# chriskery/slurm-bridge-operator

Hardware: AMD Instinct MI355X
Metric: placements/sec + job×node fit evals/sec, 100k nodes×1M jobs, 1–8 MI355X (higher is better)
Workload: dtype int32

## Files before the change

slurm-bridge-operator_amd/csrc/dev_decider_bench.hip:

```cpp
#define MW_DECIDER_BENCH 1
#include "fit_commit_mw.h"

namespace fitgpu {
__global__ __launch_bounds__(64) void k_dec_bench(int w, int32_t* out, unsigned long long* cyc) {
    extern __shared__ __attribute__((aligned(16))) unsigned char smem[];
    MwShared* S = reinterpret_cast<MwShared*>(smem);
    const int lane = threadIdx.x;
    mw_reset_items(S, threadIdx.x);
    __syncthreads();
    for (int r = 0; r < MW_R; ++r) {
        if (lane == 0) {
            S->rec[r].h = MwHdr{0u, 1, MW_M, r, 1, 1, 0, 0, 1u, 0u, KEY_INF};
        }
        if (lane < MW_M) {
            const int s = r * MW_M + lane;
            S->rec[r].it[lane] = MwItem{(uint32_t)s, (uint32_t)(lane + 1), s, s, 1000000, 1000000, 0, 0, 1u,
                                        mw_lds_addr(&S->rows[s].ver), 0xffffffffu, 1u};
            S->rows[s] = MwRow{1000000, 1000000, 0, 0, 1u, (uint32_t)s, s, 0};
        }
    }
    for (int i = lane; i < 64; i += 64) S->bitmap[i] = 0u;
    if (lane == 0) S->dn = 0ull;
    __syncthreads();
    CompPlan P{};
    P.nb = 0;
    P.ne = 2048;
    P.w = w;
    const unsigned long long t0 = __builtin_amdgcn_s_memtime();
    const CommitResult r = mw_decider(P, S, out, 1);
    const unsigned long long t1 = __builtin_amdgcn_s_memtime();
    if (lane == 0) {
        cyc[0] = t1 - t0;
        cyc[1] = r.done;
        cyc[2] = r.placed;
        cyc[3] = r.dirty;
    }
}
}

extern "C" int dec_bench(int w, unsigned long long* host_out) {
    int32_t* out;
    unsigned long long* cyc;
    if (hipMalloc(&out, sizeof(int32_t) * (w + 64)) != hipSuccess) return -1;
    if (hipMalloc(&cyc, 64) != hipSuccess) return -1;
// ... 12 lines not shown
```

slurm-bridge-operator_amd/csrc/engine.cpp:

```cpp
#include <errno.h>
#include <fcntl.h>
#include <hip/hip_runtime_api.h>
#include <hip/hip_vector_types.h>
#include <rccl/rccl.h>
#include <sys/file.h>
#include <sys/stat.h>
#include <unistd.h>

#include <algorithm>
#include <chrono>
#include <cstdarg>
#include <cstdio>
#include <cstdlib>
#include <cstring>
#include <initializer_list>
#include <map>
#include <mutex>
#include <new>
#include <string>
#include <vector>

#include "../../include/fitgpu.h"
#include "fit_device.h"

// ... 278 lines not shown
    DBuf<NodeRec> rec;
    DBuf<int32_t> col_cpu, col_mem, col_gpu, col_av, perm;
    DBuf<uint32_t> col_mask;
    DBuf<int32_t> rb_cpu, rb_mem, rb_gpu;
    std::vector<uint32_t> h_mask;
    bool have_nodes = false;
    int64_t loads = 0;

    int32_t np = 0;
    int32_t ptab[128];
    DBuf<int32_t> d_ptab;

    DBuf<int32_t> jcpu, jmem, jgpu, jwall, out, jl, jpk;
    DBuf<uint16_t> jpart, jk;
    DBuf<int8_t> jcomp;
    DBuf<uint64_t> cand, bnd;
    DBuf<JobRec> wjob;
    DBuf<CompPlan> plan;
    DBuf<CommitResult> res;
    HBuf<CompPlan> h_plan;
    HBuf<CommitResult> h_res;
    DBuf<int32_t> jls;
    HBuf<int32_t> h_jls;

    int32_t tl_slots = 0, tl_slot_min = 0;
    bool have_tl = false;
    DBuf<Seg> slab;
    DBuf<TlHdr> tlhdr;
    DBuf<int32_t> outs, rel_off, rel_slot, rel_cpu, rel_mem, rel_gpu;
    DBuf<uint32_t> tl_err;
// ... 272 lines not shown
    int rc = engine_plan(c, jb, E, (int64_t)MAX_SLICES * KS, [&](int32_t len, CompState& s) {
        for (s.ks = KS;; s.ks /= 2) {
            const int slices = MAX_SLICES * KS / s.ks;
            s.sub = std::max(MIN_SUB, (len + SCAN_WAVES * slices - 1) / (SCAN_WAVES * slices));
            s.nslice = std::max(1, (len + SCAN_WAVES * s.sub - 1) / (SCAN_WAVES * s.sub));
            if (s.sub <= sub_target || s.ks / 2 < ks_min) break;
        }
    });
    if (rc) return rc;
    size_t lds = engine_lds_bytes(E.maxnodes);
    if (const char* e = getenv("FIT_ENGINE_LDS_MIN")) lds = std::max(lds, (size_t)atol(e));
    int per_cu = engine_blocks_per_cu(lds);
    if (per_cu <= 0) return fail(FIT_E_HIP, "k_engine does not fit on a CU (lds %zu)", lds);
    int workers = std::max(8, std::max(1, per_cu - 1) * c->cus - nc);
    if (const char* e = getenv("FIT_WORKERS")) workers = std::max(1, atoi(e));
    static const bool no_backup = getenv("FIT_REC_BACKUP") && atoi(getenv("FIT_REC_BACKUP")) == 0;
    if (c->rec_bak.ensure(std::max(c->nn, 1))) return FIT_E_OOM;
    if (!no_backup)
        HIP_TRY(hipMemcpyAsync(c->rec_bak.p, c->rec.p, sizeof(NodeRec) * c->nn, hipMemcpyDeviceToDevice, st));
    return engine_launch(
        c, jb, E, workers, "placement engine",
        [&]() -> int {
            HIP_TRY(launch_engine(nc + workers, lds, st, c->ectl.p, c->ering.p, c->ecs.p, c->eco.p,
                                  c->plan.p, nc, c->rec.p, c->jl.p, cpu, mem, gpu, wall, part, nk,
                                  c->cand.p, c->bnd.p, c->wjob.p, out, kmax, c->ebusy.p, c->jpk.p,
                                  c->wd_ticks));
            return 0;
        },
        [&](int trip) -> int {
            if (!trip) return 0;
            if (no_backup) {
                c->have_nodes = c->have_tl = false;
                return trip;
            }
            HIP_TRY(hipMemcpyAsync(c->rec.p, c->rec_bak.p, sizeof(NodeRec) * c->nn, hipMemcpyDeviceToDevice, st));
            HIP_TRY(hipStreamSynchronize(st));
            return trip;
        },
        S);
}

// ... 248 lines not shown
               const SmallBatch* hb = nullptr) {
    const double t0 = now_ms();
    fit_stats S;
    memset(&S, 0, sizeof S);
    S.jobs = J;
    hipStream_t st = c->st;
    if (J <= c->small_direct && !c->collective()) {
        const int rc = place_direct(c, J, cpu, mem, gpu, wall, part, nk, kmax, out, h_out, S, hb);
        if (rc) return rc;
        if (h_out_done) *h_out_done = h_out != nullptr;
        S.unplaced = J - S.placed - S.rejected;
        S.ms_total = now_ms() - t0;
        if (stats) *stats = S;
        return 0;
    }
    if (c->jcomp.ensure(std::max(J, 1))) return FIT_E_OOM;
    HIP_TRY(launch_prefilter(st, cpu, mem, gpu, wall, part, nk, J, kmax, c->d_ptab.p, c->np, out,
                             c->jcomp.p));
    const int C = c->ncomp;
    std::vector<int32_t> jb;
    const int pre_mode = !c->collective() ? 0
                         : (c->shard_mode == FIT_SHARD_AUTO ? (C >= c->world ? FIT_SHARD_COMPONENTS : FIT_SHARD_NODES)
                                                            : c->shard_mode);
    const bool cls_able = c->cls_nodes_ok && pre_mode != FIT_SHARD_NODES;
    const bool try_cls = (c->cls_mode == 1 || c->cls_mode == 2) && cls_able && (c->cls_mode == 2 || J > c->small_batch);
    bool cls_ok = false;
    int rc0 = build_job_lists(c, J, S, jb, cpu, mem, gpu, part, try_cls, &cls_ok);
    if (rc0) return rc0;
    const int32_t live = J - S.rejected;
    if (c->cls_mode == 3 && cls_able && live > c->small_batch && 2 * (int64_t)c->last_multi >= live) {
        rc0 = classify_jobs(c, J, cpu, mem, gpu, part, &cls_ok);
        if (rc0) return rc0;
    }
// ... 1389 lines not shown
```

slurm-bridge-operator_amd/csrc/fit_commit_mw.h:

```cpp
#pragma once
#include "fit_common.h"
#include "fit_engine_ctl.h"

namespace fitgpu {

#ifndef MW_ITEMS
#define MW_ITEMS 8
#endif
constexpr int MW_M = MW_ITEMS;
constexpr int MW_R = 8;
#ifndef MW_SNAP
#define MW_SNAP MW_ITEMS
#endif
static_assert(MW_SNAP >= 1 && MW_SNAP <= MW_ITEMS, "a later snapshot only shortens the ring span");
constexpr int MW_WAVES = SCAN_WAVES;
constexpr int MW_H = MW_WAVES - 1;
static_assert(MW_M == 8, "the decider holds one item per lane of its 8-lane ring group");
static_assert(MW_R >= MW_M, "record slot reuse relies on the lag bound");

#ifndef MW_HSLEEP
#define MW_HSLEEP 1
#endif
constexpr int MW_EPL = (MAX_SLICES * KS + 63) / 64;
static_assert(MW_EPL <= 2, "at most two candidate entries per lane");

struct alignas(16) MwRow {
    int32_t cpu, mem, gpu, avail;
    uint32_t mask, pos;
    int32_t orig, ver;
};

struct alignas(16) MwItem {
    uint32_t pos, score;
    int32_t tag, orig;
    int32_t cpu, mem, gpu, avail;
    uint32_t mask;
    uint32_t chk_addr, chk_mask, chk_thr;
};

struct alignas(16) MwHdr {
    uint32_t ready;
    int32_t v, n, q;
    int32_t cpu, mem, gpu, wall;
    uint32_t pbit;
// ... 2 lines not shown
};

struct alignas(16) MwRec {
    MwHdr h;
    MwItem it[MW_M];
};

struct alignas(16) MwShared {
    uint64_t dn;
    uint32_t halt;
    uint32_t fail;
    int32_t res[4];
    uint32_t pubt;
    uint32_t wd;
    uint32_t trip_arg;
    uint32_t pad[5];
    MwRec rec[MW_R];
    MwRow rows[UCAP];
    uint32_t bitmap[1];
};

__host__ __device__ constexpr size_t mw_lds_bytes(int32_t max_component_nodes) {
    return sizeof(MwShared) + (size_t)((max_component_nodes + 31) / 32) * 4;
}

#ifdef FIT_STAMPS
constexpr int MW_NSTAMP = 24;
__device__ unsigned long long g_mw[64][MW_NSTAMP];
#define MW_CLK(v) unsigned long long v = __builtin_amdgcn_s_memtime()
#define MW_DECL(v) unsigned long long v = 0
#define MW_ACC(v, x) v += (x)
#define MW_ADD(I_, V_) do { if ((threadIdx.x & 63) == 0) atomicAdd(&g_mw[blockIdx.x & 63][I_], (unsigned long long)(V_)); } while (0)
#else
#define MW_CLK(v)
#define MW_DECL(v)
// ... 308 lines not shown
    return true;
}

template <class Q>
__device__ __forceinline__ Q* rfl_ptr(Q* p) {
    const uint64_t v = (uint64_t)(uintptr_t)p;
    return (Q*)(uintptr_t)(((uint64_t)(uint32_t)rfl((int32_t)(v >> 32)) << 32) |
                           (uint32_t)rfl((int32_t)(uint32_t)v));
}
__device__ __forceinline__ MwTiles tiles_sgpr(const MwTiles& T) {
    return MwTiles{rfl_ptr(T.tdone), (unsigned)rfl((int32_t)T.need), rfl_ptr(T.ring),
                   rfl_ptr(T.ctl), (unsigned)rfl((int32_t)T.round), (unsigned)rfl((int32_t)T.comp),
                   (unsigned)rfl((int32_t)T.ntj), rfl_ptr(T.feas)};
}

constexpr int UPL_MW = UCAP / 64;
constexpr int MW_NE = MW_EPL + UPL_MW;
static_assert(MW_NE <= 8, "entry index takes 3 bits (and 4 bits of item index each in 32)");
static_assert(MW_M <= 15, "item index + 1 fits 4 bits");
__device__ __forceinline__ uint64_t mw_tag(uint64_t k, int e) {
    return k == KEY_INF ? KEY_INF
                        : (k & 0xffffffff00000000ull) | (uint32_t)(((uint32_t)k << 3) | (uint32_t)e);
}
__device__ __forceinline__ void mw_cas(uint64_t& a, uint64_t& b) {
    const uint64_t lo = umin64(a, b), hi = umax64(a, b);
    a = lo;
    b = hi;
}
template <int N>
__device__ __forceinline__ void mw_sort(uint64_t (&q)[N]) {
    if constexpr (N == 4) {
        mw_cas(q[0], q[1]); mw_cas(q[2], q[3]);
        mw_cas(q[0], q[2]); mw_cas(q[1], q[3]);
// ... 173 lines not shown
            R_->h.v = (int32_t)v_;                                                             \
            R_->h.n = n_;                                                                      \
            R_->h.q = J_.q;                                                                    \
            lds_release();                         \
            lds_st(&R_->h.ready, (uint32_t)i + 1u);                                            \
        }                                                                                      \
        {                                                                                      \
            MW_CLK(hp1_);                                                                      \
            MW_ACC(a_hp, hp1_);                                                                \
        }                                                                                      \
        MW_ACC(a_hn, 1);                                                                       \
        MW_ACC(a_hi, n_);                                                                      \
        i += MW_H;                                                                             \
    }

__device__ __noinline__ void mw_helper(const CompPlan& Pref, MwShared* Sin,
                                       const NodeRec* __restrict__ rec_,
                                       const uint64_t* __restrict__ cand_,
                                       const uint64_t* __restrict__ bnd_,
                                       const JobRec* __restrict__ wjob_, int h, MwTiles Tin) {
    const MwTiles T = tiles_sgpr(Tin);
    const GAS NodeRec* const rec = gview(rec_);
    const GAS uint64_t* const cand = gview(cand_);
    const GAS uint64_t* const bnd = gview(bnd_);
    const GAS JobRec* const wjob = gview(wjob_);
    const CompPlan P = plan_sgpr(Pref);
    MwShared* const S = lds_opaque(Sin);
    const int lane = threadIdx.x & 63;
    const int E = P.nslice * P.ks;
    bool has[MW_EPL];
    int64_t eoff[MW_EPL];
#pragma unroll
    for (int e = 0; e < MW_EPL; ++e) {
        has[e] = lane + 64 * e < E;
        eoff[e] = P.cand_off + (has[e] ? lane + 64 * e : 0);
// ... 60 lines not shown
    v4i32 a;
    v4i32 b;
    int32_t slot;
};

typedef uint32_t v4u32 __attribute__((ext_vector_type(4)));
struct MwRecRegs {
    v4u32 h0, h1, h2;
    v4u32 i0, i1, i2;
};

struct MwDec {
    int t, nu, placed, stop;
    int done;
    bool exit;
#ifdef MW_SEGSTAMP
    unsigned long long seg[8], prev;
#endif
};
#ifdef MW_SEGSTAMP
__device__ unsigned long long g_seg[8];
#define MW_SEG(D_, i)                                                                           \
    do {                                                                                        \
        __builtin_amdgcn_sched_barrier(0);                                                      \
        unsigned long long now_;                                                                \
        asm volatile("s_memtime %0\n\ts_waitcnt lgkmcnt(0)" : "=s"(now_)::"memory");            \
        __builtin_amdgcn_sched_barrier(0);                                                      \
        if (i > 0) D_.seg[i] += now_ - D_.prev;                                                 \
        D_.prev = now_;                                                                         \
    } while (0)
// ... 11 lines not shown
    x.h1 = hp[1];
    x.h2 = hp[2];
    x.i0 = ip[0];
    x.i1 = ip[1];
    x.i2 = ip[2];
}

__device__ __forceinline__ void mw_reset_items(MwShared* S, unsigned tid) {
    static_assert(sizeof(MwItem) == 48 && offsetof(MwItem, mask) == 32, "the probe is the last 16 B");
    static_assert((MW_M & (MW_M - 1)) == 0, "item index by shift and mask");
    const uint32_t sink = mw_lds_addr(&S->pad[0]);
    for (unsigned i = tid; i < MW_R * MW_M; i += blockDim.x)
        *reinterpret_cast<v4u32*>(&S->rec[i / MW_M].it[i % MW_M].mask) = v4u32{0u, sink, 0u, 0u};
}

template <int E>
__device__ __forceinline__ void mw_decide(MwShared* S, const CompPlan& P, MwDec& D, MwRing& R,
                                          MwRecRegs& cur, MwRecRegs& nxt, uint32_t& flag,
                                          int32_t& oq, int32_t& ov, int32_t* out, int kmax,
                                          uint64_t& waitcyc) {
    const int lane = threadIdx.x & 63;
    const int t = D.t;
#ifdef MW_DECIDER_BENCH
    if (t >= P.w) D.exit = true;
#endif
    MW_SEG(D, 0);
    lds_release();
    __hip_atomic_store(&S->dn, ((uint64_t)(uint32_t)D.nu << 32) | (uint32_t)t, __ATOMIC_RELAXED,
                       __HIP_MEMORY_SCOPE_WORKGROUP);
    const MwRec* Rn = &S->rec[(E + 1) & (MW_R - 1)];
    const uint32_t flag_n = lds_ld(&Rn->h.ready);
// ... 27 lines not shown
        d.sm = (tr ? R.a.y : (int32_t)x.i1.y) - jm;
        d.sg = (tr ? R.a.z : (int32_t)x.i1.z) - jg;
        d.sa = tr ? R.a.w : (int32_t)x.i1.w;
        d.sk = tr ? R.b.x : (int32_t)x.i2.x;
        d.so = tr ? R.b.z : (int32_t)x.i0.w;
        d.ss = tr ? R.slot : (int32_t)x.i0.z;
        const uint64_t best = min8_2pass(cand);
        const uint64_t mine = __ballot(cand == best) & 0xffull;
        d.w = __builtin_ctzll(mine | 0x100ull) & 7;
        const uint32_t bhi = (uint32_t)readlane((int32_t)(best >> 32), 0);
        const uint32_t blo = (uint32_t)readlane((int32_t)(uint32_t)best, 0);
        d.bs = ((uint64_t)bhi << 32) | blo;
        d.placed = d.bs != KEY_INF;
        d.wslot = readlane(d.ss, d.w);
        d.fresh = d.placed && d.wslot < 0;
        d.full = d.fresh && D.nu >= UCAP;
        d.stopB = B != KEY_INF && d.bs > B;
        return d;
    };
    Dec d = decide(cur);
    MW_SEG(D, 2);
#ifdef MW_DECIDER_BENCH
    const bool rec_missing = false;
#else
    const bool rec_missing = flag != (uint32_t)t + 1u;
#endif
    if (__builtin_expect(!D.exit && (rec_missing || d.stopB || d.full), 0)) {
        if (rec_missing) {
            MW_CLK(c0);
            for (unsigned sp = 0;; ++sp) {
                flag = lds_ld(&S->rec[t & (MW_R - 1)].h.ready);
// ... 1 lines not shown
                if (sp > MW_SPIN_LIMIT || lds_ld(&S->fail)) {
                    lds_st(&S->fail, TRIP_DECIDER_REC);
                    D.stop = 3;
                    D.exit = true;
                    break;
                }
                __builtin_amdgcn_s_sleep(0);
            }
            lds_acquire();
            mw_read_rec(&S->rec[t & (MW_R - 1)], lane & 7, cur);
            {
                MW_CLK(c1);
                MW_ACC(waitcyc, c1 - c0);
            }
            d = decide(cur);
        }
        if (!D.exit && (d.stopB || d.full)) {
            D.done = (int32_t)cur.h2.y;
            if (D.done < P.w) D.stop = d.stopB ? 1 : 2;
            D.exit = true;
        }
    }
    MW_SEG(D, 3);
    const bool go = !D.exit;
    const bool placed = d.placed && go, fresh = d.fresh && go;
    const int w = d.w;
    const int32_t pos = (int32_t)(uint32_t)d.bs;
    const int32_t nc = readlane(d.sc, w), nm = readlane(d.sm, w), ng = readlane(d.sg, w);
    const int32_t na = readlane(d.sa, w), nk = readlane(d.sk, w), no = readlane(d.so, w);
    const int32_t slot = fresh ? D.nu : d.wslot;
// ... 34 lines not shown
            : "memory");
    }
    D.nu += fresh;
    D.placed += placed;
    MW_SEG(D, 6);
    oq = writelane(rfl((int32_t)cur.h0.w), t & 63, oq);
    ov = writelane(placed ? no : -1, t & 63, ov);
    if (E == 7 && go && (t & 63) == 63) {
        if (oq >= 0) ((GAS int32_t*)out)[(int64_t)oq * kmax] = ov;
        oq = -1;
    }
    D.t = t + (go ? 1 : 0);
    MW_SEG(D, 7);
}

__device__ __noinline__ CommitResult mw_decider(const CompPlan& Pref, MwShared* Sin,
                                                int32_t* __restrict__ out, int kmax) {
    const CompPlan P = plan_sgpr(Pref);
    MwShared* const S = lds_opaque(Sin);
    const int lane = threadIdx.x & 63;
    __builtin_amdgcn_s_setprio(3);
    MwDec D{0, 0, 0, 0, 0, false};
#ifdef MW_SEGSTAMP
    for (int i = 0; i < 8; ++i) D.seg[i] = 0;
    D.prev = 0;
#endif
    MwRing R;
    R.a = v4i32{0, 0, 0, 0};
    R.b = v4i32{0, -1, -1, -1};
    R.slot = -1;
    int32_t oq = -1, ov = -1;
    uint64_t waitcyc = 0;
    MW_CLK(d0);
    MwRecRegs ra, rb;
    uint32_t flag = 0;
    if (P.w > 0) {
        for (unsigned sp = 0;; ++sp) {
// ... 9 lines not shown
                break;
            }
            __builtin_amdgcn_s_sleep(0);
        }
        lds_acquire();
        mw_read_rec(&S->rec[0], lane & 7, ra);
    } else {
        D.exit = true;
    }
    {
        MW_CLK(r0c);
        MW_ADD(17, r0c - d0);
        MW_ADD(18, 1);
    }
    while (!D.exit) {
        mw_decide<0>(S, P, D, R, ra, rb, flag, oq, ov, out, kmax, waitcyc);
        mw_decide<1>(S, P, D, R, rb, ra, flag, oq, ov, out, kmax, waitcyc);
        mw_decide<2>(S, P, D, R, ra, rb, flag, oq, ov, out, kmax, waitcyc);
        mw_decide<3>(S, P, D, R, rb, ra, flag, oq, ov, out, kmax, waitcyc);
        mw_decide<4>(S, P, D, R, ra, rb, flag, oq, ov, out, kmax, waitcyc);
        mw_decide<5>(S, P, D, R, rb, ra, flag, oq, ov, out, kmax, waitcyc);
        mw_decide<6>(S, P, D, R, ra, rb, flag, oq, ov, out, kmax, waitcyc);
        mw_decide<7>(S, P, D, R, rb, ra, flag, oq, ov, out, kmax, waitcyc);
    }
    const int t = D.t;
    if (oq >= 0 && lane < (t & 63)) ((GAS int32_t*)out)[(int64_t)oq * kmax] = ov;
    lds_release();
    __hip_atomic_store(&S->dn, ((uint64_t)(uint32_t)D.nu << 32) | (uint32_t)t, __ATOMIC_RELAXED,
                       __HIP_MEMORY_SCOPE_WORKGROUP);
    lds_st(&S->halt, 1u);
    MW_CLK(d1);
    MW_ADD(0, d1 - d0);
#ifdef MW_SEGSTAMP
    if (lane == 0)
        for (int i = 0; i < 8; ++i) g_seg[i] = D.seg[i];
#endif
    MW_ADD(1, waitcyc);
    MW_ADD(2, t);
#ifdef MW_DECIDER_BENCH
    D.done = t;
#endif
    return CommitResult{D.done, D.stop, D.nu, D.placed};
}

// ... 1 lines not shown
                                                         NodeRec* __restrict__ rec,
                                                         const uint64_t* __restrict__ cand,
                                                         const uint64_t* __restrict__ bnd,
                                                         const JobRec* __restrict__ wjob,
                                                         int32_t* __restrict__ out, int kmax,
                                                         MwTiles T = MwTiles{nullptr, 0u, nullptr, nullptr, 0u, 0u, 0u, nullptr}) {
    const int wave = __builtin_amdgcn_readfirstlane((int)(threadIdx.x >> 6));
    const int nwords = (P.ne - P.nb + 31) >> 5;
    for (int i = threadIdx.x; i < nwords; i += MW_WAVES * 64) S->bitmap[i] = 0u;
    if (threadIdx.x < MW_R) S->rec[threadIdx.x].h.ready = 0u;
    mw_reset_items(S, threadIdx.x);
    if (threadIdx.x == 0) {
        S->dn = 0ull;
        S->halt = 0u;
        S->fail = 0u;
    }
    __syncthreads();
    if (wave == 0) {
        const CommitResult r = mw_decider(P, S, out, kmax);
        if (threadIdx.x == 0) {
            S->res[0] = r.done;
            S->res[1] = r.stop;
            S->res[2] = r.dirty;
            S->res[3] = r.placed;
        }
    } else {
        mw_helper(P, S, rec, cand, bnd, wjob, wave, T);
    }
    __syncthreads();
    const CommitResult r{S->res[0], S->res[1], S->res[2], S->res[3]};
    for (int u = threadIdx.x; u < r.dirty; u += MW_WAVES * 64) {
        const MwRow w = S->rows[u];
        NodeRec* d = rec + w.pos;
        __hip_atomic_store(reinterpret_cast<uint64_t*>(&d->cpu),
                           (uint64_t)(uint32_t)w.cpu | ((uint64_t)(uint32_t)w.mem << 32),
                           __ATOMIC_RELAXED, __HIP_MEMORY_SCOPE_AGENT);
        __hip_atomic_store(&d->gpu, w.gpu, __ATOMIC_RELAXED, __HIP_MEMORY_SCOPE_AGENT);
    }
    asm volatile("s_waitcnt vmcnt(0)" ::: "memory");
    __syncthreads();
    return r;
}

}
```

slurm-bridge-operator_amd/csrc/fit_device.h:

```cpp
#pragma once
#include <hip/hip_runtime_api.h>
#include <hip/hip_vector_types.h>
#include <stdint.h>

namespace fitgpu {

#ifndef FIT_KS
#define FIT_KS 16
#endif
constexpr int KS = FIT_KS;
static_assert(KS >= 2 && KS <= 16 && (KS & (KS - 1)) == 0, "FIT_KS must be a power of two in [2, 16]");
constexpr int SCAN_WAVES = 8;
constexpr int SCAN_JOBS = 64;
#ifndef FIT_MIN_SUB
#define FIT_MIN_SUB 64
#endif
constexpr int MIN_SUB = FIT_MIN_SUB;
#ifndef FIT_MAX_SLICES
#define FIT_MAX_SLICES (128 / FIT_KS)
#endif
constexpr int MAX_SLICES = FIT_MAX_SLICES;
#ifndef FIT_TL_KS
#define FIT_TL_KS 4
#endif
// ... 37 lines not shown
    int32_t pair_off;
};

struct CompState {
    int32_t nb, ne, sb, se, nslice, sub;
    int32_t jstart, jend;
    int64_t cand_off;
    int32_t slot0;
    int32_t wmin, wmax;
    int32_t ks;
    int64_t cand_alt;
    int32_t slot_alt;
    int32_t pair_off;
};

struct CompOut {
    int64_t evals, placed, done_jobs, rounds, stops_rescan, stops_dirty;
    int64_t t_commit, t_wait;
};

#ifndef FIT_TL_SPLIT_DEF
#define FIT_TL_SPLIT_DEF 0
#endif
constexpr int TL_MAX_SLOTS = 1024;
#ifndef TL_UCAP_DEF
#define TL_UCAP_DEF 64
#endif
constexpr int TL_UCAP = TL_UCAP_DEF;
#ifndef FIT_TL_CAND
#define FIT_TL_CAND 128
// ... 180 lines not shown
};


hipError_t launch_scan(int blocks, hipStream_t st, const NodeRec* rec, const int32_t* jl,
                       const int32_t* jcpu, const int32_t* jmem, const int32_t* jgpu,
                       const int32_t* jwall, const uint16_t* jpart, const uint16_t* jk,
                       const CompPlan* plan, int ncomp, uint64_t* cand, uint64_t* bnd,
                       JobRec* wjob);
hipError_t launch_commit(int ncomp, int epl, size_t lds_bytes, hipStream_t st, NodeRec* rec,
                         const CompPlan* plan, const uint64_t* cand, int64_t rank_stride,
                         int nranks, const uint64_t* bnd, const JobRec* wjob, int32_t* out,
                         int kmax, CommitResult* res);
hipError_t launch_prefilter(hipStream_t st, const int32_t* jcpu, const int32_t* jmem,
                            const int32_t* jgpu, const int32_t* jwall, const uint16_t* jpart, const uint16_t* jk,
                            int32_t nj, int32_t kmax, const int32_t* ptab, int32_t np,
                            int32_t* out, int8_t* jcomp);
size_t joblists_scratch_ints(int32_t nj);
hipError_t launch_joblists(hipStream_t st, const int8_t* jcomp, int32_t nj, int ncomp,
                           int32_t* scratch, int32_t* g, int32_t* jb, int32_t* mb, int32_t* jl,
                           int32_t* jpk);
hipError_t launch_small_args(hipStream_t st, int ncomp, NodeRec* rec, const SmallComps& C, const int32_t* ptab,
                             int32_t np, const SmallBatch& B, bool has_nk, int32_t nj, int32_t kmax, int32_t* out,
                             int32_t* stat);
hipError_t launch_small(hipStream_t st, int ncomp, NodeRec* rec, const SmallComps& C,
                        const int32_t* ptab, int32_t np, const int32_t* jcpu, const int32_t* jmem,
                        const int32_t* jgpu, const int32_t* jwall, const uint16_t* jpart,
                        const uint16_t* jk, int32_t nj, int32_t kmax, int32_t* out, int32_t* stat);
hipError_t launch_gather_nodes(hipStream_t st, const int32_t* cpu, const int32_t* mem,
                               const int32_t* gpu, const int32_t* av, const uint32_t* mask,
                               const int32_t* perm, int32_t nn, NodeRec* rec);
hipError_t launch_scatter_nodes(hipStream_t st, const NodeRec* rec, int32_t nn, int32_t* cpu,
// ... 12 lines not shown
                        const int16_t* jcls, const int4* dem, const int32_t* ncls, int32_t kmax, int32_t* out,
                        CompOut* co, unsigned* err);
hipError_t launch_class_out(hipStream_t st, int32_t* out, int64_t n, const NodeRec* rec);
size_t engine_ctl_bytes();
size_t engine_ctl_error_offset();
size_t engine_ctl_trip_offset();
size_t engine_ring_bytes();
size_t engine_ring_tasks();
int engine_ring_groups();
int engine_blocks_per_cu(size_t lds);
hipError_t launch_engine(int blocks, size_t lds, hipStream_t st, void* ctl, void* ring,
                         const void* cs, void* co, CompPlan* plans, int ncomp, NodeRec* rec,
                         const int32_t* jl, const int32_t* jcpu, const int32_t* jmem,
                         const int32_t* jgpu, const int32_t* jwall, const uint16_t* jpart,
                         const uint16_t* jk, uint64_t* cand, uint64_t* bnd, JobRec* wjob,
                         int32_t* out, int kmax, int64_t* wbusy, const int32_t* jpk, unsigned wd);
hipError_t launch_build_tl(hipStream_t st, const int32_t* cpu, const int32_t* mem,
                           const int32_t* gpu, const int32_t* av, const uint32_t* mask,
                           const int32_t* perm, int32_t nn, int32_t H, int32_t slot_min,
                           const int32_t* off, const int32_t* rs, const int32_t* rc,
                           const int32_t* rm, const int32_t* rg, Seg* slab, TlHdr* hdr,
                           uint32_t* err);
hipError_t launch_scan_tl(int blocks, hipStream_t st, const Seg* slab, const TlHdr* hdr,
                          const int32_t* jl, const int32_t* jcpu, const int32_t* jmem,
                          const int32_t* jgpu, const int32_t* jwall, const uint16_t* jpart,
                          const CompPlan* plan, int ncomp, uint64_t* cand, uint64_t* bnd,
                          JobRec* wjob, int32_t H, int32_t slot_min);
size_t commit_tl_lds_bytes(int32_t max_component_nodes);
int commit_tl_runs(int32_t max_component_nodes);
hipError_t launch_commit_tl(int ncomp, int epl, size_t lds, hipStream_t st, Seg* slab,
                            TlHdr* hdr, const CompPlan* plan, const uint64_t* cand,
// ... 21 lines not shown
```

slurm-bridge-operator_amd/csrc/fit_kernels.hip:

```cpp
#include "fit_common.h"

namespace fitgpu {

__global__ __launch_bounds__(SCAN_WAVES * 64) void k_scan(
    const NodeRec* __restrict__ rec, const int32_t* __restrict__ jl,
    const int32_t* __restrict__ jcpu, const int32_t* __restrict__ jmem,
    const int32_t* __restrict__ jgpu, const int32_t* __restrict__ jwall,
    const uint16_t* __restrict__ jpart, const uint16_t* __restrict__ jk,
    const CompPlan* __restrict__ plan, int ncomp, uint64_t* __restrict__ cand,
    uint64_t* __restrict__ bnd, JobRec* __restrict__ wjob) {
    __shared__ uint64_t xk[SCAN_WAVES / 2][KS][64];
    const int c = find_comp(plan, ncomp, blockIdx.x);
    const CompPlan P = plan[c];
    const int local = blockIdx.x - P.blk0;
    const int tile = __builtin_amdgcn_readfirstlane(local / P.nslice);
    const int s = __builtin_amdgcn_readfirstlane(local - tile * P.nslice);
    scan_tile<false, KS>(P, tile, s, rec, jl, jcpu, jmem, jgpu, jwall, jpart, jk, cand, bnd, wjob, xk);
}

template <int EPL>
__global__ __launch_bounds__(64) void k_commit(
    NodeRec* __restrict__ rec, const CompPlan* __restrict__ plan,
    const uint64_t* __restrict__ cand, int64_t rank_stride, int nranks,
    const uint64_t* __restrict__ bnd, const JobRec* __restrict__ wjob,
// ... 17 lines not shown
                                        bool* rej, int* k) {
    const int p = jpart[q];
    *k = jk ? max((int)jk[q], 1) : 1;
    bool r = p >= np;
    if (!r) {
        const int mt = ptab[p], mc = ptab[32 + p], mm = ptab[64 + p];
        r = (mt >= 0 && jwall[q] > mt) || (mc >= 0 && jcpu[q] > mc) || (mm >= 0 && jmem[q] > mm);
    }
    *rej = r;
    int comp = r ? -2 : ptab[96 + p];
    if (comp >= 0 && *k > 1) comp |= 0x40;
    if (*k > kmax || jcpu[q] < 0 || jmem[q] < 0 || jwall[q] < 0 || (jgpu && jgpu[q] < 0)) comp = -3;
    return comp;
}

__global__ void k_prefilter(const int32_t* __restrict__ jcpu, const int32_t* __restrict__ jmem,
                            const int32_t* __restrict__ jgpu, const int32_t* __restrict__ jwall, const uint16_t* __restrict__ jpart,
                            const uint16_t* __restrict__ jk, int32_t nj, int32_t kmax,
                            const int32_t* __restrict__ ptab ,
                            int32_t np, int32_t* __restrict__ out, int8_t* __restrict__ jcomp) {
    const int q = blockIdx.x * blockDim.x + threadIdx.x;
    if (q >= nj) return;
    bool rej;
    int k;
    jcomp[q] = (int8_t)job_code(q, jcpu, jmem, jgpu, jwall, jpart, jk, kmax, ptab, np, &rej, &k);
    for (int i = 0; i < kmax; ++i) out[(int64_t)q * kmax + i] = (rej && i < k) ? -2 : -1;
}

__global__ void k_gather_nodes(const int32_t* __restrict__ cpu, const int32_t* __restrict__ mem,
                               const int32_t* __restrict__ gpu, const int32_t* __restrict__ av,
                               const uint32_t* __restrict__ mask, const int32_t* __restrict__ perm,
                               int32_t nn, NodeRec* __restrict__ rec) {
    const int i = blockIdx.x * blockDim.x + threadIdx.x;
    if (i >= nn) return;
    const int x = perm[i];
    NodeRec r;
    r.cpu = max(cpu[x], -1);
    r.mem = max(mem[x], -1);
    r.gpu = max(gpu[x], -1);
    r.avail = max(av[x], -1);
    r.mask = mask[x];
// ... 3 lines not shown
}

__global__ void k_scatter_nodes(const NodeRec* __restrict__ rec, int32_t nn,
                                int32_t* __restrict__ cpu, int32_t* __restrict__ mem,
                                int32_t* __restrict__ gpu) {
    const int i = blockIdx.x * blockDim.x + threadIdx.x;
    if (i >= nn) return;
    const NodeRec r = rec[i];
    if (r.cpu >= 0) cpu[r.orig] = r.cpu;
    if (r.mem >= 0) mem[r.orig] = r.mem;
    if (r.gpu >= 0) gpu[r.orig] = r.gpu;
}


constexpr int JL_BLOCK = 1024;
constexpr int JL_MAXC = 32;

__global__ __launch_bounds__(JL_BLOCK) void k_jl_count(const int8_t* __restrict__ jcomp, int32_t nj,
                                                       int ncomp, int32_t* __restrict__ bc,
                                                       int32_t* __restrict__ bm,
                                                       int32_t* __restrict__ g) {
    __shared__ int32_t wc[JL_BLOCK / 64][JL_MAXC], wm[JL_BLOCK / 64][JL_MAXC];
    const int q = blockIdx.x * JL_BLOCK + threadIdx.x;
    const int wave = threadIdx.x >> 6, lane = threadIdx.x & 63;
    const int k = q < nj ? jcomp[q] : -1;
    const int comp = k >= 0 ? (k & 0x3f) : -1;
    const bool multi = k >= 0 && (k & 0x40);
    for (int cc = 0; cc < ncomp; ++cc) {
        const uint64_t m = __ballot(comp == cc), mm = __ballot(comp == cc && multi);
        if (lane == 0) {
            wc[wave][cc] = __popcll(m);
// ... 405 lines not shown
                        const uint16_t* jk, int32_t nj, int32_t kmax, int32_t* out, int32_t* stat) {
    hipLaunchKernelGGL(k_small, dim3(ncomp > 0 ? ncomp : 1), dim3(SMALL_THREADS), 0, st, rec, C, ncomp, ptab,
                       np, jcpu, jmem, jgpu, jwall, jpart, jk, nj, kmax, out, stat);
    return hipGetLastError();
}

#ifdef FIT_STAMPS
extern "C" int fit_debug_commit_stamps(unsigned long long* out ) {
    return hipMemcpyFromSymbol(out, HIP_SYMBOL(g_stamps), sizeof(g_stamps)) == hipSuccess ? 0 : -2;
}
#endif

hipError_t launch_prefilter(hipStream_t st, const int32_t* jcpu, const int32_t* jmem,
                            const int32_t* jgpu, const int32_t* jwall, const uint16_t* jpart, const uint16_t* jk,
                            int32_t nj, int32_t kmax, const int32_t* ptab, int32_t np,
                            int32_t* out, int8_t* jcomp) {
    if (nj == 0) return hipSuccess;
    hipLaunchKernelGGL(k_prefilter, dim3((nj + 255) / 256), dim3(256), 0, st, jcpu, jmem, jgpu, jwall,
                       jpart, jk, nj, kmax, ptab, np, out, jcomp);
    return hipGetLastError();
}

size_t joblists_scratch_ints(int32_t nj) { return (size_t)2 * ((nj + JL_BLOCK - 1) / JL_BLOCK) * JL_MAXC; }

hipError_t launch_joblists(hipStream_t st, const int8_t* jcomp, int32_t nj, int ncomp,
                           int32_t* scratch, int32_t* g, int32_t* jb, int32_t* mb, int32_t* jl,
                           int32_t* jpk) {
    if (ncomp > JL_MAXC) return hipErrorInvalidValue;
    const int nblocks = (nj + JL_BLOCK - 1) / JL_BLOCK;
    int32_t* bc = scratch;
    int32_t* bm = scratch + (size_t)nblocks * JL_MAXC;
    hipError_t e = hipMemsetAsync(g, 0, 2 * sizeof(int32_t), st);
    if (e != hipSuccess) return e;
    if (nj > 0) {
// ... 32 lines not shown
```

slurm-bridge-operator_amd/csrc/fit_persistent.hip:

```cpp
#include <algorithm>

#include "fit_commit_mw.h"
#include "fit_engine_ctl.h"

namespace fitgpu {

__device__ __noinline__ CommitResult engine_commit_single(int c, const CompPlan P, NodeRec* rec,
                                                          const uint64_t* cand,
                                                          const uint64_t* bnd, const JobRec* wjob,
                                                          int32_t* out, int kmax,
                                                          uint32_t* bitmap, uint32_t* scratch) {
    typedef __attribute__((address_space(3))) uint32_t* LdsWords;
    uint32_t a = (uint32_t)(uintptr_t)(LdsWords)bitmap;
    asm volatile("" : "+s"(a));
#ifdef __HIP_DEVICE_COMPILE__
#define FIT_GLOBAL(T, p) ((__attribute__((address_space(1))) T*)(p))
#else
#define FIT_GLOBAL(T, p) ((T*)(p))
#endif
    uint32_t sa = (uint32_t)(uintptr_t)(LdsWords)scratch;
    asm volatile("" : "+s"(sa));
    return commit_window<MW_EPL, true>(c, P, FIT_GLOBAL(NodeRec, rec), FIT_GLOBAL(const uint64_t, cand), 0,
                                       1, FIT_GLOBAL(const uint64_t, bnd), FIT_GLOBAL(const JobRec, wjob),
                                       FIT_GLOBAL(int32_t, out), kmax, (LdsWords)(uintptr_t)a, sa);
// ... 15 lines not shown
#ifndef K_T0PAIR
#define K_T0PAIR 1
#endif
constexpr size_t STAGE_OFF = (sizeof(uint64_t) * (SCAN_WAVES / 2) * KS * 64 + 16 + 63) & ~(size_t)63;
constexpr int STAGE_ROWS = 1024;

__global__ __launch_bounds__(SCAN_WAVES * 64) void k_engine(
    EngineCtl* __restrict__ ctl, unsigned long long* __restrict__ ring,
    const CompState* __restrict__ cs, CompOut* __restrict__ co, CompPlan* __restrict__ plans,
    int ncomp, NodeRec* __restrict__ rec, const int32_t* __restrict__ jl,
    const int32_t* __restrict__ jcpu, const int32_t* __restrict__ jmem,
    const int32_t* __restrict__ jgpu, const int32_t* __restrict__ jwall,
    const uint16_t* __restrict__ jpart, const uint16_t* __restrict__ jk,
    uint64_t* __restrict__ cand, uint64_t* __restrict__ bnd, JobRec* __restrict__ wjob,
    int32_t* __restrict__ out, int kmax, int64_t* __restrict__ wbusy,
    const int32_t* __restrict__ jpk, unsigned wd) {
    extern __shared__ __attribute__((aligned(16))) unsigned char smem[];
    const int lane = threadIdx.x & 63;
    if (threadIdx.x == 0) stamp_start(ctl);

    if ((int)blockIdx.x < ncomp) {
        __shared__ int s_fail;
        const int wave = __builtin_amdgcn_readfirstlane((int)(threadIdx.x >> 6));
        const int c = blockIdx.x;
        const CompState S = cs[c];
        MwShared* M = reinterpret_cast<MwShared*>(smem);
        if (threadIdx.x == 0) M->wd = wd;
        int32_t cursor = S.jstart, win = S.wmin;
        unsigned target[2] = {0u, 0u};
        unsigned used[2] = {0u, 0u};
        int64_t evals = 0, placed = 0, rounds = 0, sr = 0, sd = 0, tc = 0, tw = 0;
        bool prev_multi = false;
        int wide_left = 0;
        while (cursor < S.jend) {
            const int w = min(win, S.jend - cursor);
            const unsigned rnd = (unsigned)rounds + 1u;
            const int par = (int)(rnd & 1u);
            CompPlan P;
            P.nb = S.nb;
            P.ne = S.ne;
            P.sb = S.sb;
            P.se = S.se;
// ... 270 lines not shown
int engine_ring_groups() { return (int)QGROUPS; }

int engine_blocks_per_cu(size_t lds) {
    int n = 0;
    if (hipOccupancyMaxActiveBlocksPerMultiprocessor(&n, k_engine, SCAN_WAVES * 64, lds) !=
        hipSuccess)
        return 0;
    return n;
}

hipError_t launch_engine(int blocks, size_t lds, hipStream_t st, void* ctl, void* ring,
                         const void* cs, void* co, CompPlan* plans, int ncomp, NodeRec* rec,
                         const int32_t* jl, const int32_t* jcpu, const int32_t* jmem,
                         const int32_t* jgpu, const int32_t* jwall, const uint16_t* jpart,
                         const uint16_t* jk, uint64_t* cand, uint64_t* bnd, JobRec* wjob,
                         int32_t* out, int kmax, int64_t* wbusy, const int32_t* jpk, unsigned wd) {
    hipLaunchKernelGGL(k_engine, dim3(blocks), dim3(SCAN_WAVES * 64), lds, st,
                       static_cast<EngineCtl*>(ctl), static_cast<unsigned long long*>(ring),
                       static_cast<const CompState*>(cs), static_cast<CompOut*>(co), plans, ncomp,
                       rec, jl, jcpu, jmem, jgpu, jwall, jpart, jk, cand, bnd, wjob, out, kmax,
                       wbusy, jpk, wd);
    return hipGetLastError();
}

}

#ifdef FIT_TILE0_STAMPS
extern "C" int fit_debug_tile0(unsigned long long* out ) {
    return hipMemcpyFromSymbol(out, HIP_SYMBOL(fitgpu::g_tile0), sizeof(fitgpu::g_tile0)) == hipSuccess ? 0 : -2;
}
#endif
#ifdef FIT_STAMPS
extern "C" int fit_debug_commit_stamps_pe(unsigned long long* out ) {
    return hipMemcpyFromSymbol(out, HIP_SYMBOL(fitgpu::g_stamps), sizeof(fitgpu::g_stamps)) ==
                   hipSuccess ? 0 : -2;
}
// ... 6 lines not shown
```

Baseline: 38.12 million.

## Recycle dead rows in decider set using per-component minimum job demand

New measurement: 38.82 million, median of 6. 1.02x the previous value.

```diff
diff --git a/slurm-bridge-operator_amd/csrc/dev_decider_bench.hip b/slurm-bridge-operator_amd/csrc/dev_decider_bench.hip
--- a/slurm-bridge-operator_amd/csrc/dev_decider_bench.hip
+++ b/slurm-bridge-operator_amd/csrc/dev_decider_bench.hip
@@ -27,7 +27,7 @@
     P.ne = 2048;
     P.w = w;
     const unsigned long long t0 = __builtin_amdgcn_s_memtime();
-    const CommitResult r = mw_decider(P, S, out, 1);
+    const CommitResult r = mw_decider<false>(P, S, out, 1);
     const unsigned long long t1 = __builtin_amdgcn_s_memtime();
     if (lane == 0) {
         cyc[0] = t1 - t0;
diff --git a/slurm-bridge-operator_amd/csrc/engine.cpp b/slurm-bridge-operator_amd/csrc/engine.cpp
--- a/slurm-bridge-operator_amd/csrc/engine.cpp
+++ b/slurm-bridge-operator_amd/csrc/engine.cpp
@@ -316,6 +316,7 @@
     DBuf<int32_t> jcpu, jmem, jgpu, jwall, out, jl, jpk;
     DBuf<uint16_t> jpart, jk;
     DBuf<int8_t> jcomp;
+    DBuf<int32_t> jmin;
     DBuf<uint64_t> cand, bnd;
     DBuf<JobRec> wjob;
     DBuf<CompPlan> plan;
@@ -618,6 +619,9 @@
     if (per_cu <= 0) return fail(FIT_E_HIP, "k_engine does not fit on a CU (lds %zu)", lds);
     int workers = std::max(8, std::max(1, per_cu - 1) * c->cus - nc);
     if (const char* e = getenv("FIT_WORKERS")) workers = std::max(1, atoi(e));
+    EngineCompIds ids;
+    memset(&ids, 0, sizeof ids);
+    for (int i = 0; i < nc; ++i) ids.id[i] = (int8_t)E.comps[i];
     static const bool no_backup = getenv("FIT_REC_BACKUP") && atoi(getenv("FIT_REC_BACKUP")) == 0;
     if (c->rec_bak.ensure(std::max(c->nn, 1))) return FIT_E_OOM;
     if (!no_backup)
@@ -628,7 +632,7 @@
             HIP_TRY(launch_engine(nc + workers, lds, st, c->ectl.p, c->ering.p, c->ecs.p, c->eco.p,
                                   c->plan.p, nc, c->rec.p, c->jl.p, cpu, mem, gpu, wall, part, nk,
                                   c->cand.p, c->bnd.p, c->wjob.p, out, kmax, c->ebusy.p, c->jpk.p,
-                                  c->wd_ticks));
+                                  c->wd_ticks, c->jmin.p, ids));
             return 0;
         },
         [&](int trip) -> int {
@@ -907,9 +911,10 @@
         if (stats) *stats = S;
         return 0;
     }
-    if (c->jcomp.ensure(std::max(J, 1))) return FIT_E_OOM;
+    if (c->jcomp.ensure(std::max(J, 1)) || c->jmin.ensure(3 * ENGINE_MAXC)) return FIT_E_OOM;
+    HIP_TRY(hipMemsetAsync(c->jmin.p, JMIN_FILL, sizeof(int32_t) * 3 * ENGINE_MAXC, st));
     HIP_TRY(launch_prefilter(st, cpu, mem, gpu, wall, part, nk, J, kmax, c->d_ptab.p, c->np, out,
-                             c->jcomp.p));
+                             c->jcomp.p, c->jmin.p));
     const int C = c->ncomp;
     std::vector<int32_t> jb;
     const int pre_mode = !c->collective() ? 0
diff --git a/slurm-bridge-operator_amd/csrc/fit_commit_mw.h b/slurm-bridge-operator_amd/csrc/fit_commit_mw.h
--- a/slurm-bridge-operator_amd/csrc/fit_commit_mw.h
+++ b/slurm-bridge-operator_amd/csrc/fit_commit_mw.h
@@ -24,10 +24,24 @@
 constexpr int MW_EPL = (MAX_SLICES * KS + 63) / 64;
 static_assert(MW_EPL <= 2, "at most two candidate entries per lane");
 
+constexpr int MW_UCAP = 64;
+#ifndef MW_RETIRE
+#define MW_RETIRE 128
+#endif
+constexpr int MW_RCAP = MW_RETIRE;
+static_assert(UCAP == 2 * MW_UCAP, "retired[] lies over the rows a 64-row set leaves unused");
+static_assert(MW_RCAP * 16 <= (UCAP - MW_UCAP) * 32, "retired[] fits there");
+static_assert(MW_UCAP + MW_RCAP < 256, "a 256-job window of fresh nodes still fills the set");
+
 struct alignas(16) MwRow {
     int32_t cpu, mem, gpu, avail;
     uint32_t mask, pos;
     int32_t orig, ver;
+};
+
+struct alignas(16) MwRet {
+    uint32_t pos;
+    int32_t cpu, mem, gpu;
 };
 
 struct alignas(16) MwItem {
@@ -60,11 +74,19 @@
     uint32_t pubt;
     uint32_t wd;
     uint32_t trip_arg;
-    uint32_t pad[5];
+    uint32_t pad[1];
+    uint32_t nret;
+    int32_t mind[3];
+    uint32_t ucap;
+    uint32_t pad1[1];
     MwRec rec[MW_R];
     MwRow rows[UCAP];
     uint32_t bitmap[1];
 };
+
+__device__ __forceinline__ MwRet* mw_retired(MwShared* S) {
+    return reinterpret_cast<MwRet*>(&S->rows[MW_UCAP]);
+}
 
 __host__ __device__ constexpr size_t mw_lds_bytes(int32_t max_component_nodes) {
     return sizeof(MwShared) + (size_t)((max_component_nodes + 31) / 32) * 4;
@@ -403,9 +425,7 @@
                    (unsigned)rfl((int32_t)T.ntj), rfl_ptr(T.feas)};
 }
 
-constexpr int UPL_MW = UCAP / 64;
-constexpr int MW_NE = MW_EPL + UPL_MW;
-static_assert(MW_NE <= 8, "entry index takes 3 bits (and 4 bits of item index each in 32)");
+static_assert(MW_EPL + UCAP / 64 <= 8, "entry index takes 3 bits (and 4 bits of item index each in 32)");
 static_assert(MW_M <= 15, "item index + 1 fits 4 bits");
 __device__ __forceinline__ uint64_t mw_tag(uint64_t k, int e) {
     return k == KEY_INF ? KEY_INF
@@ -609,11 +629,13 @@
         i += MW_H;                                                                             \
     }
 
+template <int UPL_MW>
 __device__ __noinline__ void mw_helper(const CompPlan& Pref, MwShared* Sin,
                                        const NodeRec* __restrict__ rec_,
                                        const uint64_t* __restrict__ cand_,
                                        const uint64_t* __restrict__ bnd_,
                                        const JobRec* __restrict__ wjob_, int h, MwTiles Tin) {
+    constexpr int MW_NE = MW_EPL + UPL_MW;
     const MwTiles T = tiles_sgpr(Tin);
     const GAS NodeRec* const rec = gview(rec_);
     const GAS uint64_t* const cand = gview(cand_);
@@ -704,6 +726,8 @@
     int t, nu, placed, stop;
     int done;
     bool exit;
+    int nret;
+    uint64_t dead;
 #ifdef MW_SEGSTAMP
     unsigned long long seg[8], prev;
 #endif
@@ -745,7 +769,44 @@
         *reinterpret_cast<v4u32*>(&S->rec[i / MW_M].it[i % MW_M].mask) = v4u32{0u, sink, 0u, 0u};
 }
 
-template <int E>
+__device__ __forceinline__ int mw_recycle(MwShared* S, const CompPlan& P, MwDec& D, uint32_t pos) {
+    if (D.dead == 0ull) {
+        const int room = MW_RCAP - D.nret;
+        if (room <= 0) return -1;
+        const int lane = threadIdx.x & 63;
+        const MwRow r = S->rows[lane];
+        const int32_t mc = S->mind[0], mm = S->mind[1], mg = S->mind[2];
+        const uint64_t all = __ballot(r.cpu < mc || r.mem < mm || r.gpu < mg);
+        const int rank = (int)__builtin_amdgcn_mbcnt_hi((uint32_t)(all >> 32),
+                                                        __builtin_amdgcn_mbcnt_lo((uint32_t)all, 0u));
+        const bool mine = ((all >> lane) & 1ull) && rank < room;
+        const uint64_t dm = __ballot(mine);
+        if (dm == 0ull) return -1;
+        if (mine) mw_retired(S)[D.nret + rank] = MwRet{r.pos, r.cpu, r.mem, r.gpu};
+        D.nret += (int)__builtin_popcountll(dm);
+        D.dead = dm;
+        __builtin_amdgcn_s_waitcnt(0xc07f);
+    }
+    const int s = (int)__builtin_ctzll(D.dead);
+    D.dead &= D.dead - 1ull;
+    {
+        const uint32_t rel = pos - (uint32_t)P.nb;
+        const uint32_t ba = mw_lds_addr(&S->bitmap[rel >> 5]);
+        const uint32_t bv = 1u << (rel & 31);
+        uint64_t sv;
+        asm volatile(
+            "s_mov_b64 %[sv], exec\n\t"
+            "s_mov_b64 exec, 1\n\t"
+            "ds_or_b32 %[ba], %[bv]\n\t"
+            "s_mov_b64 exec, %[sv]"
+            : [sv] "=&s"(sv)
+            : [ba] "v"(ba), [bv] "v"(bv)
+            : "memory");
+    }
+    return s;
+}
+
+template <int E, bool RC>
 __device__ __forceinline__ void mw_decide(MwShared* S, const CompPlan& P, MwDec& D, MwRing& R,
                                           MwRecRegs& cur, MwRecRegs& nxt, uint32_t& flag,
                                           int32_t& oq, int32_t& ov, int32_t* out, int kmax,
@@ -803,7 +864,7 @@
         d.placed = d.bs != KEY_INF;
         d.wslot = readlane(d.ss, d.w);
         d.fresh = d.placed && d.wslot < 0;
-        d.full = d.fresh && D.nu >= UCAP;
+        d.full = d.fresh && D.nu >= (RC ? MW_UCAP : UCAP);
         d.stopB = B != KEY_INF && d.bs > B;
         return d;
     };
@@ -835,6 +896,16 @@
                 MW_ACC(waitcyc, c1 - c0);
             }
             d = decide(cur);
+        }
+        if constexpr (RC && MW_RCAP > 0) {
+            if (!D.exit && d.full && !d.stopB) {
+                const int s = mw_recycle(S, P, D, (uint32_t)d.bs);
+                if (s >= 0) {
+                    d.wslot = s;
+                    d.fresh = false;
+                    d.full = false;
+                }
+            }
         }
         if (!D.exit && (d.stopB || d.full)) {
             D.done = (int32_t)cur.h2.y;
@@ -899,13 +970,14 @@
     MW_SEG(D, 7);
 }
 
+template <bool RC>
 __device__ __noinline__ CommitResult mw_decider(const CompPlan& Pref, MwShared* Sin,
                                                 int32_t* __restrict__ out, int kmax) {
     const CompPlan P = plan_sgpr(Pref);
     MwShared* const S = lds_opaque(Sin);
     const int lane = threadIdx.x & 63;
     __builtin_amdgcn_s_setprio(3);
-    MwDec D{0, 0, 0, 0, 0, false};
+    MwDec D{0, 0, 0, 0, 0, false, 0, 0ull};
 #ifdef MW_SEGSTAMP
     for (int i = 0; i < 8; ++i) D.seg[i] = 0;
     D.prev = 0;
@@ -945,20 +1017,21 @@
         MW_ADD(18, 1);
     }
     while (!D.exit) {
-        mw_decide<0>(S, P, D, R, ra, rb, flag, oq, ov, out, kmax, waitcyc);
-        mw_decide<1>(S, P, D, R, rb, ra, flag, oq, ov, out, kmax, waitcyc);
-        mw_decide<2>(S, P, D, R, ra, rb, flag, oq, ov, out, kmax, waitcyc);
-        mw_decide<3>(S, P, D, R, rb, ra, flag, oq, ov, out, kmax, waitcyc);
-        mw_decide<4>(S, P, D, R, ra, rb, flag, oq, ov, out, kmax, waitcyc);
-        mw_decide<5>(S, P, D, R, rb, ra, flag, oq, ov, out, kmax, waitcyc);
-        mw_decide<6>(S, P, D, R, ra, rb, flag, oq, ov, out, kmax, waitcyc);
-        mw_decide<7>(S, P, D, R, rb, ra, flag, oq, ov, out, kmax, waitcyc);
+        mw_decide<0, RC>(S, P, D, R, ra, rb, flag, oq, ov, out, kmax, waitcyc);
+        mw_decide<1, RC>(S, P, D, R, rb, ra, flag, oq, ov, out, kmax, waitcyc);
+        mw_decide<2, RC>(S, P, D, R, ra, rb, flag, oq, ov, out, kmax, waitcyc);
+        mw_decide<3, RC>(S, P, D, R, rb, ra, flag, oq, ov, out, kmax, waitcyc);
+        mw_decide<4, RC>(S, P, D, R, ra, rb, flag, oq, ov, out, kmax, waitcyc);
+        mw_decide<5, RC>(S, P, D, R, rb, ra, flag, oq, ov, out, kmax, waitcyc);
+        mw_decide<6, RC>(S, P, D, R, ra, rb, flag, oq, ov, out, kmax, waitcyc);
+        mw_decide<7, RC>(S, P, D, R, rb, ra, flag, oq, ov, out, kmax, waitcyc);
     }
     const int t = D.t;
     if (oq >= 0 && lane < (t & 63)) ((GAS int32_t*)out)[(int64_t)oq * kmax] = ov;
     lds_release();
     __hip_atomic_store(&S->dn, ((uint64_t)(uint32_t)D.nu << 32) | (uint32_t)t, __ATOMIC_RELAXED,
                        __HIP_MEMORY_SCOPE_WORKGROUP);
+    lds_st(&S->nret, (uint32_t)D.nret);
     lds_st(&S->halt, 1u);
     MW_CLK(d1);
     MW_ADD(0, d1 - d0);
@@ -990,10 +1063,12 @@
         S->dn = 0ull;
         S->halt = 0u;
         S->fail = 0u;
+        S->nret = 0u;
     }
     __syncthreads();
     if (wave == 0) {
-        const CommitResult r = mw_decider(P, S, out, kmax);
+        const CommitResult r = S->ucap == (uint32_t)MW_UCAP ? mw_decider<true>(P, S, out, kmax)
+                                                            : mw_decider<false>(P, S, out, kmax);
         if (threadIdx.x == 0) {
             S->res[0] = r.done;
             S->res[1] = r.stop;
@@ -1001,7 +1076,8 @@
             S->res[3] = r.placed;
         }
     } else {
-        mw_helper(P, S, rec, cand, bnd, wjob, wave, T);
+        if (S->ucap == (uint32_t)MW_UCAP) mw_helper<1>(P, S, rec, cand, bnd, wjob, wave, T);
+        else mw_helper<2>(P, S, rec, cand, bnd, wjob, wave, T);
     }
     __syncthreads();
     const CommitResult r{S->res[0], S->res[1], S->res[2], S->res[3]};
@@ -1013,6 +1089,14 @@
                            __ATOMIC_RELAXED, __HIP_MEMORY_SCOPE_AGENT);
         __hip_atomic_store(&d->gpu, w.gpu, __ATOMIC_RELAXED, __HIP_MEMORY_SCOPE_AGENT);
     }
+    for (int u = threadIdx.x; u < (int)S->nret; u += MW_WAVES * 64) {
+        const MwRet w = mw_retired(S)[u];
+        NodeRec* d = rec + w.pos;
+        __hip_atomic_store(reinterpret_cast<uint64_t*>(&d->cpu),
+                           (uint64_t)(uint32_t)w.cpu | ((uint64_t)(uint32_t)w.mem << 32),
+                           __ATOMIC_RELAXED, __HIP_MEMORY_SCOPE_AGENT);
+        __hip_atomic_store(&d->gpu, w.gpu, __ATOMIC_RELAXED, __HIP_MEMORY_SCOPE_AGENT);
+    }
     asm volatile("s_waitcnt vmcnt(0)" ::: "memory");
     __syncthreads();
     return r;
diff --git a/slurm-bridge-operator_amd/csrc/fit_device.h b/slurm-bridge-operator_amd/csrc/fit_device.h
--- a/slurm-bridge-operator_amd/csrc/fit_device.h
+++ b/slurm-bridge-operator_amd/csrc/fit_device.h
@@ -75,6 +75,12 @@
     int32_t pair_off;
 };
 
+constexpr int ENGINE_MAXC = 32;
+constexpr int JMIN_FILL = 0x7f;
+struct EngineCompIds {
+    int8_t id[ENGINE_MAXC];
+};
+
 struct CompOut {
     int64_t evals, placed, done_jobs, rounds, stops_rescan, stops_dirty;
     int64_t t_commit, t_wait;
@@ -285,7 +291,7 @@
 hipError_t launch_prefilter(hipStream_t st, const int32_t* jcpu, const int32_t* jmem,
                             const int32_t* jgpu, const int32_t* jwall, const uint16_t* jpart, const uint16_t* jk,
                             int32_t nj, int32_t kmax, const int32_t* ptab, int32_t np,
-                            int32_t* out, int8_t* jcomp);
+                            int32_t* out, int8_t* jcomp, int32_t* jmin = nullptr);
 size_t joblists_scratch_ints(int32_t nj);
 hipError_t launch_joblists(hipStream_t st, const int8_t* jcomp, int32_t nj, int ncomp,
                            int32_t* scratch, int32_t* g, int32_t* jb, int32_t* mb, int32_t* jl,
@@ -328,7 +334,8 @@
                          const int32_t* jl, const int32_t* jcpu, const int32_t* jmem,
                          const int32_t* jgpu, const int32_t* jwall, const uint16_t* jpart,
                          const uint16_t* jk, uint64_t* cand, uint64_t* bnd, JobRec* wjob,
-                         int32_t* out, int kmax, int64_t* wbusy, const int32_t* jpk, unsigned wd);
+                         int32_t* out, int kmax, int64_t* wbusy, const int32_t* jpk, unsigned wd,
+                         const int32_t* jmin, const EngineCompIds& ids);
 hipError_t launch_build_tl(hipStream_t st, const int32_t* cpu, const int32_t* mem,
                            const int32_t* gpu, const int32_t* av, const uint32_t* mask,
                            const int32_t* perm, int32_t nn, int32_t H, int32_t slot_min,
diff --git a/slurm-bridge-operator_amd/csrc/fit_kernels.hip b/slurm-bridge-operator_amd/csrc/fit_kernels.hip
--- a/slurm-bridge-operator_amd/csrc/fit_kernels.hip
+++ b/slurm-bridge-operator_amd/csrc/fit_kernels.hip
@@ -55,17 +55,43 @@
     return comp;
 }
 
-__global__ void k_prefilter(const int32_t* __restrict__ jcpu, const int32_t* __restrict__ jmem,
-                            const int32_t* __restrict__ jgpu, const int32_t* __restrict__ jwall, const uint16_t* __restrict__ jpart,
-                            const uint16_t* __restrict__ jk, int32_t nj, int32_t kmax,
-                            const int32_t* __restrict__ ptab ,
-                            int32_t np, int32_t* __restrict__ out, int8_t* __restrict__ jcomp) {
+template <bool MIN>
+__global__ __launch_bounds__(256) void k_prefilter(
+    const int32_t* __restrict__ jcpu, const int32_t* __restrict__ jmem,
+    const int32_t* __restrict__ jgpu, const int32_t* __restrict__ jwall, const uint16_t* __restrict__ jpart,
+    const uint16_t* __restrict__ jk, int32_t nj, int32_t kmax,
+    const int32_t* __restrict__ ptab ,
+    int32_t np, int32_t* __restrict__ out, int8_t* __restrict__ jcomp, int32_t* __restrict__ jmin) {
+    __shared__ int32_t smin[MIN ? 3 * ENGINE_MAXC : 1];
+    if constexpr (MIN) {
+        if (threadIdx.x < 3 * ENGINE_MAXC) smin[threadIdx.x] = INT32_MAX;
+        __syncthreads();
+    }
     const int q = blockIdx.x * blockDim.x + threadIdx.x;
-    if (q >= nj) return;
-    bool rej;
-    int k;
-    jcomp[q] = (int8_t)job_code(q, jcpu, jmem, jgpu, jwall, jpart, jk, kmax, ptab, np, &rej, &k);
-    for (int i = 0; i < kmax; ++i) out[(int64_t)q * kmax + i] = (rej && i < k) ? -2 : -1;
+    if (q < nj) {
+        bool rej;
+        int k;
+        const int code = job_code(q, jcpu, jmem, jgpu, jwall, jpart, jk, kmax, ptab, np, &rej, &k);
+        jcomp[q] = (int8_t)code;
+        for (int i = 0; i < kmax; ++i) out[(int64_t)q * kmax + i] = (rej && i < k) ? -2 : -1;
+        if constexpr (MIN) {
+            if (code >= 0) {
+                const int cc = code & 0x3f;
+                atomicMin(&smin[3 * cc], jcpu[q]);
+                atomicMin(&smin[3 * cc + 1], jmem[q]);
+                atomicMin(&smin[3 * cc + 2], jgpu ? jgpu[q] : 0);
+            }
+        }
+    }
+    if constexpr (MIN) {
+        __syncthreads();
+        if (threadIdx.x < 3 * ENGINE_MAXC) {
+            const int32_t v = smin[threadIdx.x];
+            if (v != INT32_MAX &&
+                v < __hip_atomic_load(&jmin[threadIdx.x], __ATOMIC_RELAXED, __HIP_MEMORY_SCOPE_AGENT))
+                atomicMin(&jmin[threadIdx.x], v);
+        }
+    }
 }
 
 __global__ void k_gather_nodes(const int32_t* __restrict__ cpu, const int32_t* __restrict__ mem,
@@ -99,7 +125,7 @@
 
 
 constexpr int JL_BLOCK = 1024;
-constexpr int JL_MAXC = 32;
+constexpr int JL_MAXC = ENGINE_MAXC;
 
 __global__ __launch_bounds__(JL_BLOCK) void k_jl_count(const int8_t* __restrict__ jcomp, int32_t nj,
                                                        int ncomp, int32_t* __restrict__ bc,
@@ -535,10 +561,14 @@
 hipError_t launch_prefilter(hipStream_t st, const int32_t* jcpu, const int32_t* jmem,
                             const int32_t* jgpu, const int32_t* jwall, const uint16_t* jpart, const uint16_t* jk,
                             int32_t nj, int32_t kmax, const int32_t* ptab, int32_t np,
-                            int32_t* out, int8_t* jcomp) {
+                            int32_t* out, int8_t* jcomp, int32_t* jmin) {
     if (nj == 0) return hipSuccess;
-    hipLaunchKernelGGL(k_prefilter, dim3((nj + 255) / 256), dim3(256), 0, st, jcpu, jmem, jgpu, jwall,
-                       jpart, jk, nj, kmax, ptab, np, out, jcomp);
+    if (jmin)
+        hipLaunchKernelGGL(k_prefilter<true>, dim3((nj + 255) / 256), dim3(256), 0, st, jcpu, jmem, jgpu,
+                           jwall, jpart, jk, nj, kmax, ptab, np, out, jcomp, jmin);
+    else
+        hipLaunchKernelGGL(k_prefilter<false>, dim3((nj + 255) / 256), dim3(256), 0, st, jcpu, jmem, jgpu,
+                           jwall, jpart, jk, nj, kmax, ptab, np, out, jcomp, jmin);
     return hipGetLastError();
 }
 
diff --git a/slurm-bridge-operator_amd/csrc/fit_persistent.hip b/slurm-bridge-operator_amd/csrc/fit_persistent.hip
--- a/slurm-bridge-operator_amd/csrc/fit_persistent.hip
+++ b/slurm-bridge-operator_amd/csrc/fit_persistent.hip
@@ -53,7 +53,8 @@
     const uint16_t* __restrict__ jpart, const uint16_t* __restrict__ jk,
     uint64_t* __restrict__ cand, uint64_t* __restrict__ bnd, JobRec* __restrict__ wjob,
     int32_t* __restrict__ out, int kmax, int64_t* __restrict__ wbusy,
-    const int32_t* __restrict__ jpk, unsigned wd) {
+    const int32_t* __restrict__ jpk, unsigned wd, const int32_t* __restrict__ jmin,
+    const EngineCompIds ids) {
     extern __shared__ __attribute__((aligned(16))) unsigned char smem[];
     const int lane = threadIdx.x & 63;
     if (threadIdx.x == 0) stamp_start(ctl);
@@ -64,7 +65,14 @@
         const int c = blockIdx.x;
         const CompState S = cs[c];
         MwShared* M = reinterpret_cast<MwShared*>(smem);
-        if (threadIdx.x == 0) M->wd = wd;
+        if (threadIdx.x == 0) {
+            M->wd = wd;
+            const int32_t* mn = jmin + 3 * ids.id[c];
+            M->mind[0] = mn[0];
+            M->mind[1] = mn[1];
+            M->mind[2] = mn[2];
+            M->ucap = S.ks == KS ? (uint32_t)MW_UCAP : (uint32_t)UCAP;
+        }
         int32_t cursor = S.jstart, win = S.wmin;
         unsigned target[2] = {0u, 0u};
         unsigned used[2] = {0u, 0u};
@@ -365,12 +373,13 @@
                          const int32_t* jl, const int32_t* jcpu, const int32_t* jmem,
                          const int32_t* jgpu, const int32_t* jwall, const uint16_t* jpart,
                          const uint16_t* jk, uint64_t* cand, uint64_t* bnd, JobRec* wjob,
-                         int32_t* out, int kmax, int64_t* wbusy, const int32_t* jpk, unsigned wd) {
+                         int32_t* out, int kmax, int64_t* wbusy, const int32_t* jpk, unsigned wd,
+                         const int32_t* jmin, const EngineCompIds& ids) {
     hipLaunchKernelGGL(k_engine, dim3(blocks), dim3(SCAN_WAVES * 64), lds, st,
                        static_cast<EngineCtl*>(ctl), static_cast<unsigned long long*>(ring),
                        static_cast<const CompState*>(cs), static_cast<CompOut*>(co), plans, ncomp,
                        rec, jl, jcpu, jmem, jgpu, jwall, jpart, jk, cand, bnd, wjob, out, kmax,
-                       wbusy, jpk, wd);
+                       wbusy, jpk, wd, jmin, ids);
     return hipGetLastError();
 }
 
```
